# physiii/radio-mapper

Measured on AMD Instinct MI355X. Metric: IQ samples cross-correlated per second, higher is better.
Workload: dtype f32; 1 GPU; cfg3: 8 buoys (28 pairs), 10 MS/s complex64, N=4096-sample windows (L=8192), 4096 windows per GPU resident in HBM; n_buoys=8, n_pairs=28, n_samples=4096, windows_per_gpu=4096, channels=1, windows_total=4096, parallelism=windows sharded x1, no collective

## Files before the change

### radio-mapper_amd/csrc/host_plan.hpp

```cpp
#pragma once
#include <climits>
#include <cmath>
#include <cstdint>
#include <cstdio>
#include <cstring>
#include <map>
#include <mutex>
#include <string>
#include <vector>

namespace rmx {

struct PairItem {
    int i, j, out, run;
};

namespace host {

struct OptionSpec {
    const char* key;
    long lo, hi;
    const char* what;
};
inline const std::vector<OptionSpec>& option_specs() {
    static const std::vector<OptionSpec> s = {
        {"stag", 0, 5, "N = 4096 fused kernel: which waves run the two halves between barriers in the opposite order (default 1)"},
        {"ncus", 1, 4096, "persistent workgroups of the fused N = 4096 kernel (default: one per CU)"},
        {"chunk_windows", 1, 1 << 20, "windows per chunk of the unfused N = 4096 path"},
        {"small4096", 0, 1, "0: N = 4096 through the fused kernel however few the windows (default 1: few windows through the per-transform kernels)"},
        {"generic4096", 0, 1, "1: N = 4096 through the generic whole-window kernels instead of k_win"},
        {"small_maxl", 256, 16384, "largest zero-padded length that runs as one LDS transform per workgroup (default 8192)"},
        {"logl1", 4, 10, "four-step: log2 of the column length"},
        {"wfused", 0, 1, "0: never g_win_fused (<= 4 buoys, N = 256 ... 2048)"},
        {"wscr", 0, 2, "g_win_scr: 0 never, 2 also for batches that do not fill the chip"},
        {"wscr14", 0, 1, "0: N = 8192 with 1024 threads x one butterfly instead of 512 x two"},
        {"wscr_per_cu", 1, 8, "persistent g_win_scr workgroups per CU"},
        {"rows_anchor", 0, 64, "four-step inverse rows: 0 never g_rows_anchor, n = from n buoys on (default 6)"},
        {"fused", 0, 2, "four-step, <= 4 buoys: 0 always the two-kernel row passes, 2 g_rows_fused for any batch size"},
        {"fused_def", 0, 1, "0: the run-time pair loop of g_rows_fused also for the default plan"},
        {"gen_chunk", 1, 4096, "generic path: at most n windows per chunk of kernel launches"},
        {"rows_tpr", 1, 1024, "four-step: threads per row (selects the run-time-length row kernels)"},
        {"cols_threads", 64, 1024, "four-step: threads per column tile"},
        {"col_logt", 3, 5, "four-step: log2 columns per tile"},
        {"kwin16k", 0, 2, "N = 16384: 1 (default) k16_fwd + k16_pairs (four quarter transforms on the fused N = 4096 network) unless wscr = 2, 2 always, 0 g_win_eo15 / the four-step kernels"},
        {"k16_min_windows", 1, 1 << 30, "kwin16k = 1: smallest batch that takes k16_fwd / k16_pairs (default: 100 / (buoys + pairs), rounded up)"},
        {"kwin8k", 0, 2, "N = 8192, batches that fill the chip: 1 (default) k_win8kl (the bin-parity halves on the fused N = 4096 network, one anchor half in LDS), 0 g_win_scr14, 2 k_win8k (-DRMX_EXPERIMENTS builds only)"},
#ifdef RMX_EXPERIMENTS
        {"pk", 0, 1, "1: k_winp (packed fp32 build of the fused kernel; -DRMX_EXPERIMENTS builds only)"},
        {"win8", 0, 1, "1: k_win8 (8 points x 1024 threads; -DRMX_EXPERIMENTS builds only)"},
#endif
    };
    return s;
}

struct Knobs {
    std::map<std::string, long> v;
    bool get(const char* key, long* out) const {
        auto it = v.find(key);
        if (it == v.end()) return false;
        *out = it->second;
        return true;
    }
    long get_or(const char* key, long dflt) const {
        long x;
        return get(key, &x) ? x : dflt;
    }
};
inline std::mutex& knob_mutex() { static std::mutex m; return m; }
inline Knobs& default_knobs() { static Knobs k; return k; }

inline int set_default_option(const char* key, long value, std::string* err) {
    if (!key) { if (err) *err = "NULL key"; return -1; }
    for (const OptionSpec& s : option_specs()) {
        if (std::strcmp(s.key, key) != 0) continue;
        std::lock_guard<std::mutex> g(knob_mutex());
        if (value == LONG_MIN) { default_knobs().v.erase(key); return 0; }
        if (value < s.lo || value > s.hi) {
            if (err) { char b[160]; std::snprintf(b, sizeof b, "option '%s': %ld not in %ld..%ld", key, value, s.lo, s.hi); *err = b; }
            return -1;
// ... 45 lines not shown
    return kBandOk;
}

struct PairPlan {
    std::vector<int32_t> pairs;
    std::vector<PairItem> items;
    std::vector<int> part_begin;
    int n_parts = 0;
    bool all_pairs = false;
};

inline bool is_default_list(int n_buoys, const int32_t* pairs, int n_pairs) {
    if (n_pairs != (long)n_buoys * (n_buoys - 1) / 2) return false;
    int q = 0;
    for (int i = 0; pairs && i < n_buoys; ++i)
        for (int j = i + 1; j < n_buoys; ++j, ++q)
            if (pairs[2 * q] != i || pairs[2 * q + 1] != j) return false;
    return true;
}

inline int make_pair_plan(int n_buoys, const int32_t* pairs, int n_pairs, int pairs_per_block, PairPlan* out, std::string* err) {
    char b[200];
    const long all = (long)n_buoys * (n_buoys - 1) / 2;
    if (n_pairs < 0) { std::snprintf(b, sizeof b, "n_pairs %d < 0", n_pairs); *err = b; return -1; }
    std::vector<int32_t> pl;
    if (pairs) {
        pl.assign(pairs, pairs + 2 * (size_t)n_pairs);
    } else {
        if (n_pairs != all) { std::snprintf(b, sizeof b, "pairs == NULL needs n_pairs == %ld, got %d", all, n_pairs); *err = b; return -1; }
        pl.reserve(2 * (size_t)all);
        for (int i = 0; i < n_buoys; ++i)
            for (int j = i + 1; j < n_buoys; ++j) { pl.push_back(i); pl.push_back(j); }
    }
    for (int q = 0; q < n_pairs; ++q) {
        const int i = pl[2 * q], j = pl[2 * q + 1];
        if (i < 0 || j < 0 || i >= n_buoys || j >= n_buoys) {
            std::snprintf(b, sizeof b, "pair %d = (%d,%d) out of range for %d buoys", q, i, j, n_buoys);
            *err = b;
            return -1;
        }
    }
    out->items.resize(n_pairs);
    for (int q = 0; q < n_pairs; ++q) out->items[q] = PairItem{pl[2 * q], pl[2 * q + 1], q, 1};
    for (int q = n_pairs - 2; q >= 0; --q)
        if (out->items[q].i == out->items[q + 1].i) out->items[q].run = out->items[q + 1].run + 1;
    const int ppb = pairs_per_block > 0 ? pairs_per_block : 7;
    const int n_parts = n_pairs > 0 ? (n_pairs + ppb - 1) / ppb : 0;
    out->part_begin.assign(n_parts + 1, 0);
    for (int k = 0; k <= n_parts && n_parts > 0; ++k) out->part_begin[k] = (int)((long)k * n_pairs / n_parts);
    out->n_parts = n_parts;
    out->all_pairs = is_default_list(n_buoys, pl.data(), n_pairs);
    out->pairs.swap(pl);
    return 0;
}

inline long generic_chunk_windows(int n_buoys, long L, int max_windows, long budget_bytes, long cap) {
    const long all_pairs = (long)n_buoys * (n_buoys - 1) / 2;
    const long per_win = (long)(n_buoys + all_pairs) * L * 8;
    long chunk = per_win > 0 ? budget_bytes / per_win : 1;
    if (chunk < 1) chunk = 1;
    if (chunk > max_windows) chunk = max_windows;
    if (chunk > 4096) chunk = 4096;
    if (cap >= 1 && cap < chunk) chunk = cap;
    return chunk;
}

constexpr long kGenericBudgetBytes = 32L << 30;
constexpr long kGenericMaxChunk = 4096;
constexpr long kMaxGridY = 65535;
struct BandsPlan {
    long chunk = 0;
    long vwindows = 0;
    long slots = 0;
    size_t prod_bytes = 0;
    size_t rec_bytes = 0;
    size_t halo_bytes = 0;
    size_t out_elems = 0;
};
inline BandsPlan plan_bands(long chunk, long n_windows, int n_bands, int n_buoys, int n_pairs, long L, bool four_step, long col_tiles,
                            int logL1, size_t rec_size, long budget_bytes = kGenericBudgetBytes, long max_vwindows = kGenericMaxChunk) {
    BandsPlan b;
    const long nb = n_bands > 0 ? n_bands : 1, np = n_pairs > 0 ? n_pairs : 0;
    if (chunk < 1) chunk = 1;
    if (nb > 1) {
        if (chunk * nb > max_vwindows) chunk = max_vwindows / nb;
        if (four_step) {
            const long per_win = ((long)n_buoys + nb * np) * L * 8;
            if (per_win > 0 && chunk > budget_bytes / per_win) chunk = budget_bytes / per_win;
            if (np > 0 && chunk * nb * np > kMaxGridY) chunk = kMaxGridY / (nb * np);
        }
        if (chunk < 1) chunk = 1;
    }
    b.chunk = chunk;
    b.vwindows = chunk * nb;
    b.slots = b.vwindows * np;
    if (four_step) {
        b.prod_bytes = (size_t)b.slots * (size_t)L * 8;
        b.rec_bytes = (size_t)b.slots * (size_t)col_tiles * rec_size;
        b.halo_bytes = ((size_t)b.slots * (size_t)col_tiles * 2 * sizeof(float)) << logL1;
    }
    b.out_elems = (size_t)(n_windows > 0 ? n_windows : 0) * (size_t)nb * (size_t)np;
    return b;
}

inline double fused_cost4096(int n_cus, int n_buoys, int n_pairs, long n_windows) {
    const long cus = n_cus > 0 ? n_cus : 1;
// ... 155 lines not shown
```

### radio-mapper_amd/csrc/kwin.hpp

```cpp
#pragma once
#include <hip/hip_runtime.h>

#include <cmath>
#include <type_traits>
#include <vector>

#include "fft_r16.hpp"
#include "lag_bounds.hpp"

namespace rmx {

using u32x4 = unsigned int __attribute__((ext_vector_type(4)));
using u32x2 = unsigned int __attribute__((ext_vector_type(2)));
using f32x4 = float __attribute__((ext_vector_type(4)));
using f32x2 = float __attribute__((ext_vector_type(2)));

constexpr int kLdsXchg = kXchgF2 * 8;
constexpr int kLdsTw2 = 16 * kTw2RowF2 * 8;
constexpr int kLdsRed = 64;
constexpr int kLdsBytes = kLdsXchg + kLdsTw2 + kLdsRed;

__device__ __forceinline__ void load_tw2_to_lds(float2* tw2_lds, const float2* __restrict__ tw2_g, int t) {
    if (t < 256) tw2_lds[(t >> 4) * kTw2RowF2 + (t & 15)] = tw2_g[t];
}
// ... 41 lines not shown
    const int g = lane >> 3, r = lane & 7;
    const bool act = g < cnt;
    const int slot = (first + g) & (kResSlots - 1);
    const float* rf = reinterpret_cast<const float*>(red) + 4 * (slot * 8 + r);
    const int* ri = reinterpret_cast<const int*>(rf);
    const float ex = act ? rf[0] : -3.0f;
    const int k = act ? ri[1] : 0x7fffffff;
    const float tm = rf[2], tp = rf[3];
    const int out = oidx[slot];
    float gmax = ex;
    gmax = fmaxf(gmax, __builtin_bit_cast(float, dpp_i<0xB1>(__builtin_bit_cast(int, gmax))));
    gmax = fmaxf(gmax, __builtin_bit_cast(float, dpp_i<0x4E>(__builtin_bit_cast(int, gmax))));
    gmax = fmaxf(gmax, __builtin_bit_cast(float, dpp_i<0x141>(__builtin_bit_cast(int, gmax))));
    int kstar = (ex == gmax) ? k : 0x7fffffff;
    kstar = min(kstar, dpp_i<0xB1>(kstar));
    kstar = min(kstar, dpp_i<0x4E>(kstar));
    kstar = min(kstar, dpp_i<0x141>(kstar));
    const bool win = act && ex == gmax && k == kstar;
    auto halo_tap = [&](int kk) -> float {
        kk = kk < 0 ? 0 : (kk > 2 * kM - 2 ? 2 * kM - 2 : kk);
        int tt, q;
        k_to_owner(kk, tt, q);
        const int ln = tt & 63;
        const int row = ln < 2 ? ln : (ln >= 62 ? ln - 60 : 0);
        return halo[(((slot * 8 + (tt >> 6)) * kHaloRows) + row) * 16 + q];
    };
    const int kc = win ? k : (kM - 1);
    const float hm = halo_tap(kc - 1), hp = halo_tap(kc + 1);
    const float b = sqrtf(fmaxf(ex, 0.0f)) * out_scale;
    const float a = sqrtf(tm >= 0.0f ? tm : hm) * out_scale;
    const float c = sqrtf(tp >= 0.0f ? tp : hp) * out_scale;
    const double den = (double)a - 2.0 * (double)b + (double)c;
    float frac = 0.0f;
    if constexpr (BOUNDED) {
        int klo = 0, khi = 0;
        if (act) lag_window(lb, w, out, kM - 1, klo, khi);
        if (kc > klo && kc < khi && den != 0.0) frac = (float)(0.5 * ((double)a - (double)c) / den);
    } else {
        if (kc > 0 && kc < 2 * kM - 2 && den != 0.0) frac = (float)(0.5 * ((double)a - (double)c) / den);
    }
    if (win) {
        lag_int[obase + out] = kc - (kM - 1);
        lag_frac[obase + out] = frac;
        peak[obase + out] = b;
    }
}

template <bool U8>
__global__ __launch_bounds__(kThreads, 2) void k_win(const void* __restrict__ iq_v, float4* __restrict__ spec,
                                                     const float4* __restrict__ tw1_g,
                                                     const float2* __restrict__ tw2_g, int n_buoys,
                                                     long first_window, float out_scale,
                                                     int* __restrict__ lag_int, float* __restrict__ lag_frac,
                                                     float* __restrict__ peak, int n_win, int , int stag) {
    constexpr bool BOUNDED = false;
    constexpr LagBounds lb{nullptr, 0, 0, 0};
#include "kwin_body.hpp"
}

template <bool U8>
__global__ __launch_bounds__(kThreads, 2) void k_win_lb(const void* __restrict__ iq_v, float4* __restrict__ spec,
                                                        const float4* __restrict__ tw1_g,
                                                        const float2* __restrict__ tw2_g, int n_buoys,
                                                        long first_window, float out_scale,
                                                        int* __restrict__ lag_int, float* __restrict__ lag_frac,
                                                        float* __restrict__ peak, int n_win, int , int stag, LagBounds lb) {
    constexpr bool BOUNDED = true;
#include "kwin_body.hpp"
}

constexpr int kTw1ScaleLog2 = 6;
constexpr double kTw1Scale = 1.0 / (1 << kTw1ScaleLog2);
inline void build_tables(std::vector<float4>& tw1, std::vector<float2>& tw2) {
    const double two_pi = 6.283185307179586476925286766559;
    tw1.resize(8 * kThreads);
    std::vector<float2> t1(16 * kThreads);
    for (int t = 0; t < kThreads; ++t) {
        const int p = t & 1, u = t >> 1;
        for (int k0 = 0; k0 < 16; ++k0) {
            double ang = -two_pi * (double)((u * k0) % kM) / (double)kM;
            if (p) ang += -two_pi * (double)u / (double)kL;
            t1[k0 * kThreads + t] = make_float2((float)(std::cos(ang) * kTw1Scale), (float)(std::sin(ang) * kTw1Scale));
        }
    }
    for (int j = 0; j < 8; ++j)
        for (int t = 0; t < kThreads; ++t) {
            const float2 a = t1[(2 * j) * kThreads + t], b = t1[(2 * j + 1) * kThreads + t];
            tw1[j * kThreads + t] = make_float4(a.x, a.y, b.x, b.y);
        }
    tw2.resize(256);
    for (int a = 0; a < 16; ++a)
        for (int b = 0; b < 16; ++b) {
            const double ang = -two_pi * (double)((a * b) % 256) / 256.0;
            tw2[a * 16 + b] = make_float2((float)std::cos(ang), (float)std::sin(ang));
        }
}

}
```

### radio-mapper_amd/csrc/kwin_body.hpp

```cpp
    extern __shared__ __attribute__((aligned(16))) char smem[];
    float2* img0 = reinterpret_cast<float2*>(smem);
    float2* img1 = reinterpret_cast<float2*>(smem + kLdsWinImg);
    float2* tw2_lds = reinterpret_cast<float2*>(smem + kLdsWinTw2);
    float* halo = reinterpret_cast<float*>(smem + kLdsWinHalo);
    float4* red = reinterpret_cast<float4*>(smem + kLdsWinRed);
    int* oidx = reinterpret_cast<int*>(smem + kLdsWinOidx);

    const int t = threadIdx.x;
    const int p = t & 1, u = t >> 1;
    const int lane = t & 63, wave = t >> 6;
    const int B = n_buoys;
    const int n_pairs = B * (B - 1) / 2;

    load_tw2_to_lds_grouped(tw2_lds, tw2_g, t);
    float2 tw1[16];
    load_tw1(tw1, tw1_g, t);
    const float4* tw2row = reinterpret_cast<const float4*>(tw2_lds + (t & 15) * kTw2RowF2);
    const int loc_m0[2] = {__builtin_amdgcn_readfirstlane(wave * kLocWave),
                           __builtin_amdgcn_readfirstlane(kLdsWinImg + wave * kLocWave)};
    const int loc_rd = wave * kLocWave + loc_read_off(lane);
    const float sgn = p ? -1.0f : 1.0f;
    const int kbase = p ? (u - 1) : (u + kM - 1);
    const int hl = lane < 2 ? lane : lane - 60;
    const bool is_halo = lane < 2 || lane >= 62;
// ... 233 lines not shown
        }
        const int qsel = min(min(qa, qb), min(qc, qd));
        const int kq = kbase + qsel * 256;
        const int wi = __builtin_bit_cast(int, wrow);
        const float wmax = fmaxf(fmaxf(__builtin_bit_cast(float, __builtin_amdgcn_readlane(wi, 0)),
                                       __builtin_bit_cast(float, __builtin_amdgcn_readlane(wi, 16))),
                                 fmaxf(__builtin_bit_cast(float, __builtin_amdgcn_readlane(wi, 32)),
                                       __builtin_bit_cast(float, __builtin_amdgcn_readlane(wi, 48))));
        const unsigned long long hit = __ballot(tmax == wmax);
        int kw, ls, qs;
        if (__popcll(hit) == 1) {
            ls = __ffsll((long long)hit) - 1;
            kw = __builtin_amdgcn_readlane(kq, ls);
            qs = __builtin_amdgcn_readlane(qsel, ls);
        } else {
            kw = wave_min_i32(tmax == wmax ? kq : 0x7fffffff);
            int ts;
            k_to_owner(kw, ts, qs);
            ls = ts & 63;
        }
        typedef float f16v __attribute__((ext_vector_type(16)));
        const f16v mv = {mag[0], mag[1], mag[2],  mag[3],  mag[4],  mag[5],  mag[6],  mag[7],
                         mag[8], mag[9], mag[10], mag[11], mag[12], mag[13], mag[14], mag[15]};
        const float sel = mv[__builtin_amdgcn_readfirstlane(qs)];
        const int seli = __builtin_bit_cast(int, sel);
        const float tapm = ls >= 2 ? __builtin_bit_cast(float, __builtin_amdgcn_readlane(seli, ls >= 2 ? ls - 2 : 0)) : -2.0f;
        const float tapp = ls <= 61 ? __builtin_bit_cast(float, __builtin_amdgcn_readlane(seli, ls <= 61 ? ls + 2 : 63)) : -2.0f;
        if (lane == 0) {
            const u32x4 rec = {__float_as_uint(wmax), (unsigned)kw, __float_as_uint(tapm), __float_as_uint(tapp)};
            *reinterpret_cast<u32x4*>(red + rb * 8 + wave) = rec;
            if (wave == 0) oidx[rb] = out_idx;
        }
        ++npend;
        ++npair;
    };
    auto pair = [&](const C16& a, const C16& s, int out_idx, auto prefetch) __attribute__((always_inline)) {
        pair_h1(a, s, seq, prefetch);
        barrier_hook(false);
        pair_h2(seq, out_idx);
        ++seq;
    };
    auto out_of = [&](int i, int j) -> int { return i * B - (i * (i + 1)) / 2 + (j - i - 1); };

    load_x(sa, 0);
    if (B > 1) load_x(sb, 1);
    cvt_x(sa);
    fwd(sa);
    for (int e = 1; e + 1 < B; ++e) {
        cvt_x(sb);
        fwd(sb);
        store_spec(sb, e);
        pair(sa, sb, out_of(0, e), [&](auto part) __attribute__((always_inline)) { load_x_part(sb, e + 1, part); });
    }
    if (B > 1) {
        cvt_x(sb);
        fwd(sb);
        store_spec(sb, B - 1);
        pair(sa, sb, out_of(0, B - 1), [&](auto part) __attribute__((always_inline)) {
            if (B > 2) {
                load_spec_part(sa, 1, part);
                load_spec_part(sb, B - 1, part);
            }
        });
    }
    {
        const int M2 = (B - 1) * (B - 2) / 2;
        const bool late_h2 = stag == 1 ? ((wave >> 1) & 1) : stag == 2 ? (wave & 1) : stag == 3 ? (wave >> 2) :
                             stag == 4 ? ((wave ^ (wave >> 2)) & 1) : (stag == 5);
        auto j_of = [&](int i, int s) -> int { return (i & 1) ? (B - 1 - s) : (i + 1 + s); };
        int ci = 1, cs = 0;
        int ni = 1, ns = 1;
        if (ns >= B - 1 - ni) { ++ni; ns = 0; }
        auto h1_of = [&](int hi, int hs, int tr) __attribute__((always_inline)) {
            int pi = hi, ps = hs + 1;
            if (ps >= B - 1 - pi) { ++pi; ps = 0; }
            const bool valid = pi + 1 < B;
            const bool new_anchor = valid && pi != hi;
            const int pj = valid ? j_of(pi, ps) : B - 1;
            pair_h1(sa, sb, tr, [&](auto part) __attribute__((always_inline)) {
                if constexpr (decltype(part)::value == 0) {
                    if (new_anchor) {
                        load_spec_part(sa, pi, std::integral_constant<int, 0>{});
                        load_spec_part(sa, pi, std::integral_constant<int, 1>{});
                        load_spec_part(sa, pi, std::integral_constant<int, 2>{});
                        load_spec_part(sa, pi, std::integral_constant<int, 3>{});
                        load_spec_part(sa, pi, std::integral_constant<int, 4>{});
                        load_spec_part(sa, pi, std::integral_constant<int, 5>{});
                        load_spec_part(sa, pi, std::integral_constant<int, 6>{});
                        load_spec_part(sa, pi, std::integral_constant<int, 7>{});
                    }
                }
                load_spec_part(sb, pj, part);
            });
        };
        if (M2 > 0) h1_of(ci, cs, seq);
        for (int m = 0; m < M2; ++m) {
            barrier_hook(false);
            const bool has_next = m + 1 < M2;
            const int out_idx = out_of(ci, j_of(ci, cs));
            if (wave >= 4) __builtin_amdgcn_s_setprio(1);
            if (late_h2) {
                if (has_next) h1_of(ni, ns, seq + 1);
                if (wave >= 4) __builtin_amdgcn_s_setprio(0);
                pair_h2(seq, out_idx);
            } else {
                pair_h2(seq, out_idx);
                if (wave >= 4) __builtin_amdgcn_s_setprio(0);
                if (has_next) h1_of(ni, ns, seq + 1);
            }
            ++seq;
            ci = ni; cs = ns;
            ++ns;
            if (ns >= B - 1 - ni) { ++ni; ns = 0; }
        }
    }
    seq = 0;
    barrier_hook(true);
    }
```

### radio-mapper_amd/csrc/rmx_hip.hip

```cpp
#include <hip/hip_runtime.h>

#include <cmath>
#include <cstdarg>
#include <cstdio>
#include <cstdlib>
#include <cstring>
#include <new>
#include <string>
#include <type_traits>
#include <utility>
#include <vector>

#include "../../include/rmx.h"
#include "host_plan.hpp"
#include "lag_bounds.hpp"
#include "xspec_weight.hpp"
#include "xspec_bands.hpp"
#include "integrate.hpp"
#include "refine.hpp"
#include "quality.hpp"
#include "fft_r16.hpp"
#include "kwin.hpp"
#include "fft_r8.hpp"
#ifdef RMX_EXPERIMENTS
// ... 3 lines not shown
#include "generic_path.hpp"
#include "win_eo.hpp"
#include "pair4096.hpp"
#include "kwin8k.hpp"
#include "kwin16k.hpp"
#ifdef RMX_EXPERIMENTS
#include "../../tools/experiments/kwin8k.hpp"
#endif
#include "caf_select.hpp"
#include "solve_path.hpp"
#include "detect_path.hpp"

struct rmx_ctx {
    struct DevStage {
        int32_t* h = nullptr;  size_t h_elems = 0;
        int* d = nullptr;      size_t d_elems = 0;
        hipEvent_t ev = nullptr;
    };
    struct GenericKernels {
        decltype(&rmx::gen::g_cols_inv<4>) cols_inv = nullptr;
        decltype(&rmx::gen::g_cols_inv<4, 0, rmx::LagBounds>) cols_inv_lb = nullptr;
        decltype(&rmx::gen::g_cols_inv<4, 0, rmx::LagBounds, rmx::Integrate>) cols_inv_int = nullptr;
        decltype(&rmx::gen::g_cols_fwd<false, 4>) cols_fwd[2] = {nullptr, nullptr};
        decltype(&rmx::gen::g_rows<true, false>) rows_fwd = nullptr;
        decltype(&rmx::gen::g_rows<true, false, false, 0, rmx::XWeight>) rows_fwd_wt = nullptr;
        decltype(&rmx::gen::g_rows<false, true, true>) rows_inv = nullptr;
        decltype(&rmx::gen::g_rows<false, true, true, 0, rmx::BandSet>) rows_inv_bs = nullptr;
        decltype(&rmx::gen::g_rows_anchor<9>) rows_anchor = nullptr;
        decltype(&rmx::gen::g_rows_fused<2, 9>) fused = nullptr;
        decltype(&rmx::gen::g_rows_fused<2, 9>) fused_def = nullptr;
        decltype(&rmx::gen::g_win_fused<2, 9, false, false>) wf[2][2] = {{nullptr, nullptr}, {nullptr, nullptr}};
        size_t wf_lds[2] = {0, 0};
        decltype(&rmx::gen::g_win_scr<9, false>) ws[2] = {nullptr, nullptr};
        decltype(&rmx::gen::g_win_eo15<false>) ws15[2] = {nullptr, nullptr};
        size_t ws_lds = 0;
        int ws_thr = 0, ws_upw = 0;
    };

    rmx::host::Knobs knobs;
    int device = 0;
    int n_cus = 256;
    int n_buoys = 0, n_samples = 0, max_windows = 0;
    hipStream_t stream = nullptr;
    bool own_stream = false;
    int chunk_windows = 0;
    int pairs_per_block = 7;
    bool ppb_user = false;
    bool small_batch = true;
    bool timing = false;
    bool resident = true;
    int pk = 0;
    int win8 = 0;
    int stag = 1;
    float4* d_tw1_8 = nullptr;
    float2* d_tb8 = nullptr;
    float2* d_tc8 = nullptr;
    bool fused = true;
    float4* d_spec = nullptr;
    float4* d_tw1 = nullptr;
    float2* d_tw2 = nullptr;
    rmx::PairItem* d_items = nullptr;
    int* d_part_begin = nullptr;
    void* d_in = nullptr;      size_t d_in_bytes = 0;
    int* d_lag = nullptr;      float* d_frac = nullptr;  float* d_peak = nullptr;  size_t d_out_elems = 0;
    int* d_dop = nullptr;
    float* d_quality = nullptr;  size_t d_quality_elems = 0;
    void* h_out = nullptr;     size_t h_out_bytes = 0;
    size_t spec_bytes = 0, scratch_bytes = 0;
    bool generic = false;
    int g_logL = 0, g_logL1 = 0, g_logL2 = 0, g_lo_bits = 0, g_chunk = 0;
    size_t g_dyn_bytes = 0, g_pair_bytes = 0;
    GenericKernels gk;
    bool g_fused = false;
    bool g_fused_always = false;
    bool g_wfused = false;
    bool g_wscr = false;
    bool g_wscr_always = false;
    int g_ws_grid = 0;
    float4* g_ws_scratch = nullptr;
    float2* g_tw_win = nullptr;
    float2* g_tw_l = nullptr;
    bool g_k8 = false;
    int g_k8_kind = 1;
    float4* g_k8_tw1 = nullptr;
    float2* g_k8_tw2 = nullptr;
    int g_k16 = 0;
    float4* g_k16_tw1 = nullptr;
    float2 *g_k16_gq = nullptr, *g_k16_tw2 = nullptr, *g_k16_tws = nullptr;
    int g_rows_anchor_min_b = 6;
    float2 *g_tw = nullptr, *g_tw1 = nullptr, *g_tw2 = nullptr, *g_thi = nullptr, *g_tlo = nullptr;
    float2 *g_spec = nullptr, *g_spec_r = nullptr, *g_prod = nullptr;
    rmx::gen::GTile* g_rec = nullptr;
    float* g_halo = nullptr;
    rmx::gen::GPair* g_pairs = nullptr;
    long g_slots_alloc = 0;
    int g_pairs_n = -1;
    std::vector<int32_t> g_pairs_plan;
    hipStream_t copy_stream = nullptr;
    hipEvent_t copy_ev[4] = {nullptr, nullptr, nullptr, nullptr};
    float2* dt_tw = nullptr;  int dt_logn = 0;  float* dt_pdb = nullptr;  size_t dt_pdb_bytes = 0;
    void* dt_in = nullptr;  size_t dt_in_bytes = 0;  void* dt_out = nullptr;  size_t dt_out_bytes = 0;
    double* sv_buoys = nullptr;  int* sv_pairs = nullptr;  size_t sv_pairs_cap = 0;
    void* sv_in = nullptr;  size_t sv_in_bytes = 0;  void* sv_out = nullptr;  size_t sv_out_bytes = 0;
    float4* d_spec_r = nullptr;  size_t spec_r_bytes = 0;
    float2* caf_rot = nullptr;  size_t caf_rot_elems = 0;
    int* caf_lag = nullptr;  float* caf_frac = nullptr;  float* caf_peak = nullptr;  int* caf_dop = nullptr;
    size_t caf_out_elems = 0;
    float* caf_nb = nullptr;  size_t caf_nb_elems = 0;
    std::vector<double> caf_grid;
    DevStage lb_stage, band_stage;
    rmx::RefPair* rf_pairs = nullptr;
    std::vector<int32_t> rf_pairs_plan;
    std::vector<int32_t> plan_pairs;
// ... 959 lines not shown
    {
        std::string why;
        if (host::check_create_args(n_buoys, n_samples, max_windows, &why) != 0) return fail(nullptr, RMX_E_INVAL, "%s", why.c_str());
    }
    int ndev = rmx_device_count();
    if (ndev <= 0) return fail(nullptr, RMX_E_NODEV, "no HIP device visible");
    if (device_id < 0 || device_id >= ndev) return fail(nullptr, RMX_E_INVAL, "device_id %d not in 0..%d", device_id, ndev - 1);
    rmx_ctx* c = new (std::nothrow) rmx_ctx();
    if (!c) return fail(nullptr, RMX_E_NOMEM, "host allocation failed");
    c->knobs = host::snapshot_default_options();
    c->device = device_id;
    c->n_buoys = n_buoys;
    c->n_samples = n_samples;
    c->max_windows = max_windows;
    int rc = RMX_OK;
    auto bail = [&](int code) {
        g_create_error = c->err;
        rmx_destroy(c);
        return code;
    };
    auto init = [&]() -> int {
        RMX_HIP(c, hipSetDevice(device_id));
        {
            int ncu = 0;
            if (hipDeviceGetAttribute(&ncu, hipDeviceAttributeMultiprocessorCount, device_id) == hipSuccess && ncu > 0)
                c->n_cus = ncu;
            { long v; if (c->knobs.get("ncus", &v) && v > 0 && v < c->n_cus) c->n_cus = (int)v; }
        }
        RMX_HIP(c, hipStreamCreateWithFlags(&c->stream, hipStreamNonBlocking));
        c->own_stream = true;
        if (n_samples != kM || c->knobs.get_or("generic4096", 0) != 0) return rmx::generic_init(c);
        int chunk = (int)c->knobs.get_or("chunk_windows", 4096);
        if (chunk < 8) chunk = 8;
        chunk = (chunk + 7) & ~7;
        if (chunk > max_windows) chunk = max_windows;
        {
            const long per_win = (long)n_buoys * (8 * kThreads) * (long)sizeof(float4);
            const long cap = (8L << 30) / per_win;
            if (chunk > cap) chunk = (int)(cap > 8 ? (cap & ~7L) : 8);
        }
        c->chunk_windows = chunk;
        {
            const int wg = chunk < c->n_cus ? chunk : c->n_cus;
            c->spec_bytes = (size_t)wg * n_buoys * (8 * kThreads) * sizeof(float4);
        }
        RMX_HIP(c, hipMalloc((void**)&c->d_spec, c->spec_bytes));
        std::vector<float4> tw1;
        std::vector<float2> tw2;
        build_tables(tw1, tw2);
        RMX_HIP(c, hipMalloc((void**)&c->d_tw1, tw1.size() * sizeof(float4)));
        RMX_HIP(c, hipMalloc((void**)&c->d_tw2, tw2.size() * sizeof(float2)));
        RMX_HIP(c, hipMemcpy(c->d_tw1, tw1.data(), tw1.size() * sizeof(float4), hipMemcpyHostToDevice));
        RMX_HIP(c, hipMemcpy(c->d_tw2, tw2.data(), tw2.size() * sizeof(float2), hipMemcpyHostToDevice));
        c->scratch_bytes = c->spec_bytes + tw1.size() * sizeof(float4) + tw2.size() * sizeof(float2);
        c->stag = (int)c->knobs.get_or("stag", 1);
        c->small_batch = c->knobs.get_or("small4096", 1) != 0;
#ifdef RMX_EXPERIMENTS
        {
            std::vector<float4> t1;
            std::vector<float2> tb, tc;
            build_tables8(t1, tb, tc);
            RMX_HIP(c, hipMalloc((void**)&c->d_tw1_8, t1.size() * sizeof(float4)));
            RMX_HIP(c, hipMalloc((void**)&c->d_tb8, tb.size() * sizeof(float2)));
            RMX_HIP(c, hipMalloc((void**)&c->d_tc8, tc.size() * sizeof(float2)));
            RMX_HIP(c, hipMemcpy(c->d_tw1_8, t1.data(), t1.size() * sizeof(float4), hipMemcpyHostToDevice));
            RMX_HIP(c, hipMemcpy(c->d_tb8, tb.data(), tb.size() * sizeof(float2), hipMemcpyHostToDevice));
            RMX_HIP(c, hipMemcpy(c->d_tc8, tc.data(), tc.size() * sizeof(float2), hipMemcpyHostToDevice));
            c->scratch_bytes += t1.size() * sizeof(float4) + (tb.size() + tc.size()) * sizeof(float2);
            int rc_x = allow_lds(c, w8::kLdsWin8Bytes, w8::k_win8<false>, w8::k_win8<true>);
            if (rc_x == RMX_OK) rc_x = allow_lds(c, pk::kLdsWinpBytes, k_winp<false>, k_winp<true>);
            if (rc_x != RMX_OK) return rc_x;
            c->pk = (int)c->knobs.get_or("pk", 0);
            c->win8 = (int)c->knobs.get_or("win8", 0);
        }
#endif
        int rc_l = allow_lds(c, kLdsBytes, k_fwd<false>, k_fwd<true>, k_fwd<false, XWeight>, k_fwd<true, XWeight>, k_pair_str<>,
                             k_pair_str<LagBounds>, k_pair_str<BandSet>, k_pair_str<LagBounds, BandSet>);
        if (rc_l == RMX_OK)
            rc_l = allow_lds(c, kLdsResBytes, k_pair_res<>, k_pair_res<LagBounds>, k_pair_res<BandSet>, k_pair_res<LagBounds, BandSet>);
        if (rc_l == RMX_OK) rc_l = allow_lds(c, kLdsWinBytes, k_win<false>, k_win<true>, k_win_lb<false>, k_win_lb<true>);
        return rc_l;
    };
    rc = init();
    if (rc != RMX_OK) return bail(rc);
    *out = c;
    return RMX_OK;
}

void rmx_destroy(rmx_ctx* c) {
    if (!c) return;
    (void)hipSetDevice(c->device);
    if (c->stream) (void)hipStreamSynchronize(c->stream);
    for (hipEvent_t e : c->ev) (void)hipEventDestroy(e);
    for (void* p : {(void*)c->g_tw, (void*)c->g_tw1, (void*)c->g_tw2, (void*)c->g_thi, (void*)c->g_tlo, (void*)c->g_spec,
                    (void*)c->g_spec_r, (void*)c->g_prod, (void*)c->g_rec, (void*)c->g_halo, (void*)c->g_pairs,
                    (void*)c->g_ws_scratch, (void*)c->g_tw_win, (void*)c->g_tw_l, (void*)c->g_k8_tw1, (void*)c->g_k8_tw2,
                    (void*)c->g_k16_tw1, (void*)c->g_k16_gq, (void*)c->g_k16_tw2, (void*)c->g_k16_tws})
        if (p) (void)hipFree(p);
    if (c->copy_stream) (void)hipStreamDestroy(c->copy_stream);
    for (hipEvent_t e : c->copy_ev)
        if (e) (void)hipEventDestroy(e);
    for (void* p : {(void*)c->dt_tw, (void*)c->dt_pdb, c->dt_in, c->dt_out})
        if (p) (void)hipFree(p);
    for (void* p : {(void*)c->sv_buoys, (void*)c->sv_pairs, c->sv_in, c->sv_out})
        if (p) (void)hipFree(p);
    for (void* p : {(void*)c->d_spec_r, (void*)c->caf_rot, (void*)c->caf_lag, (void*)c->caf_frac, (void*)c->caf_peak,
                    (void*)c->caf_dop, (void*)c->caf_nb})
        if (p) (void)hipFree(p);
    if (c->d_spec) (void)hipFree(c->d_spec);
    if (c->d_tw1) (void)hipFree(c->d_tw1);
    if (c->d_tw2) (void)hipFree(c->d_tw2);
    for (void* p : {(void*)c->d_tw1_8, (void*)c->d_tb8, (void*)c->d_tc8})
        if (p) (void)hipFree(p);
    if (c->d_items) (void)hipFree(c->d_items);
    if (c->d_part_begin) (void)hipFree(c->d_part_begin);
    if (c->d_in) (void)hipFree(c->d_in);
    if (c->d_lag) (void)hipFree(c->d_lag);
    if (c->h_out) (void)hipHostFree(c->h_out);
    if (c->rf_pairs) (void)hipFree(c->rf_pairs);
    if (c->d_quality) (void)hipFree(c->d_quality);
    for (DevStage* s : {&c->lb_stage, &c->band_stage}) {
        if (s->d) (void)hipFree(s->d);
        if (s->h) (void)hipHostFree(s->h);
        if (s->ev) (void)hipEventDestroy(s->ev);
    }
    if (c->own_stream && c->stream) (void)hipStreamDestroy(c->stream);
    delete c;
}

int rmx_set_stream(rmx_ctx* c, void* hip_stream) {
    if (!c) return RMX_E_INVAL;
    RMX_HIP(c, hipSetDevice(c->device));
    if (c->stream) RMX_HIP(c, hipStreamSynchronize(c->stream));
    if (c->own_stream && c->stream) (void)hipStreamDestroy(c->stream);
    c->stream = (hipStream_t)hip_stream;
    c->own_stream = false;
    return RMX_OK;
}

int rmx_set_default_option(const char* key, long value) {
    std::string why;
    if (host::set_default_option(key, value, &why) != 0) return fail(nullptr, RMX_E_INVAL, "%s", why.c_str());
    return RMX_OK;
}

void rmx_clear_default_options(void) { host::clear_default_options(); }

int rmx_set_option(rmx_ctx* c, const char* key, long value) {
    if (!c || !key) return RMX_E_INVAL;
    if (!strcmp(key, "chunk_windows")) {
        if (c->generic) return RMX_OK;
        long chunk = value < 8 ? 8 : value;
        chunk = (chunk + 7) & ~7L;
        if (chunk > c->max_windows) chunk = c->max_windows;
        {
            const long per_win = (long)c->n_buoys * (8 * kThreads) * (long)sizeof(float4);
            const long cap = (8L << 30) / per_win;
            if (chunk > cap) chunk = cap > 8 ? (cap & ~7L) : 8;
        }
        c->chunk_windows = (int)chunk;
        return RMX_OK;
    }
    if (!strcmp(key, "pairs_per_block")) {
        if (value < 1 || value > 1 << 20) return fail(c, RMX_E_INVAL, "pairs_per_block %ld out of range", value);
        c->pairs_per_block = (int)value;
        c->ppb_user = true;
        return RMX_OK;
    }
    if (!strcmp(key, "dbg")) {
        return fail(c, RMX_E_UNSUPPORTED, "option 'dbg': the timing-only ablation build was removed");
    }
    if (!strcmp(key, "pk") || !strcmp(key, "win8")) {
#ifdef RMX_EXPERIMENTS
        (key[0] == 'p' ? c->pk : c->win8) = value != 0;
        return RMX_OK;
#else
        return fail(c, RMX_E_UNSUPPORTED, "option '%s' exists only in the -DRMX_EXPERIMENTS build (k_win8 / k_winp)", key);
#endif
    }
    if (!strcmp(key, "stag")) {
        if (value < 0 || value > 5) return fail(c, RMX_E_INVAL, "stag %ld not in 0..5", value);
        c->stag = (int)value;
        return RMX_OK;
    }
    if (!strcmp(key, "small4096")) {
        c->small_batch = value != 0;
        return RMX_OK;
    }
    if (!strcmp(key, "fused")) {
        c->fused = value != 0;
        return RMX_OK;
    }
    if (!strcmp(key, "resident")) {
        c->resident = value != 0;
        return RMX_OK;
    }
    if (!strcmp(key, "timing")) {
        c->timing = value != 0;
        return RMX_OK;
    }
    return fail(c, RMX_E_INVAL, "unknown option '%s'", key);
}

static int ensure_spec(rmx_ctx* c, long windows) {
    const size_t nb = (size_t)windows * c->n_buoys * (8 * kThreads) * sizeof(float4);
    if (nb <= c->spec_bytes) return RMX_OK;
    RMX_HIP(c, hipStreamSynchronize(c->stream));
    float4* nspec = nullptr;
    RMX_HIP(c, hipMalloc((void**)&nspec, nb));
    (void)hipFree(c->d_spec);
    c->d_spec = nspec;
    c->scratch_bytes += nb - c->spec_bytes;
    c->spec_bytes = nb;
    return RMX_OK;
}

static constexpr size_t kPackedOutMax = 256 * 1024;
static int ensure_out(rmx_ctx* c, size_t out_elems) {
    if (c->d_out_elems >= out_elems) return RMX_OK;
    if (c->d_lag) (void)hipFree(c->d_lag);
    c->d_lag = nullptr; c->d_frac = nullptr; c->d_peak = nullptr; c->d_out_elems = 0;
    const size_t stride = (out_elems + 63) & ~(size_t)63;
    RMX_HIP(c, hipMalloc((void**)&c->d_lag, 4 * stride * sizeof(float)));
    c->d_frac = reinterpret_cast<float*>(c->d_lag) + stride;
    c->d_peak = c->d_frac + stride;
    c->d_dop = reinterpret_cast<int*>(c->d_peak + stride);
    c->d_out_elems = out_elems;
    return RMX_OK;
}
static int fetch_out(rmx_ctx* c, size_t out_elems, int32_t* lag_int, float* lag_frac, float* peak, int32_t* dop = nullptr) {
    const size_t nb = out_elems * sizeof(float);
    const char* last = reinterpret_cast<char*>(dop ? (void*)c->d_dop : (void*)c->d_peak);
    const size_t span = (size_t)(last - reinterpret_cast<char*>(c->d_lag)) + nb;
    if (span <= kPackedOutMax) {
        if (c->h_out_bytes < span) {
// ... 139 lines not shown
            RMX_HIP(c, hipStreamWaitEvent(c->copy_stream, c->copy_ev[3], 0));
        } else {
            RMX_HIP(c, hipMemcpyAsync(c->d_in, iq, in_bytes, hipMemcpyHostToDevice, c->stream));
        }
        d_iq = c->d_in;
    }
    int* d_lag = lag_int;
    float *d_frac = lag_frac, *d_peak = peak;
    const size_t out_elems = (size_t)(n_windows / call.integ) * n_pairs * (size_t)rq.n_bands;
    if (!out_dev) {
        rc = ensure_out(c, out_elems);
        if (rc == RMX_OK && call.qualified()) rc = ensure_quality(c, 4 * out_elems);
        if (rc != RMX_OK) return rc;
        d_lag = c->d_lag; d_frac = c->d_frac; d_peak = c->d_peak;
        if (call.qualified()) call.quality = c->d_quality;
    }
    auto done = [&](int rc_k) -> int {
        if (rc_k != RMX_OK || out_dev) return rc_k;
        if (call.qualified())
            RMX_HIP(c, hipMemcpyAsync(req.quality, c->d_quality, 4 * out_elems * sizeof(float), hipMemcpyDeviceToHost, c->stream));
        return fetch_out(c, out_elems, lag_int, lag_frac, peak);
    };
    if (c->generic) return done(rmx::generic_batch(c, call, caps, rq, plan, d_iq, d_lag, d_frac, d_peak, u8));
    const bool k_win_route = plan.route == host::kRouteKWin;
    const long chunk_w = n_windows < c->chunk_windows ? n_windows : c->chunk_windows;
    rc = ensure_spec(c, k_win_route ? (chunk_w < c->n_cus ? chunk_w : c->n_cus) : chunk_w);
    if (rc != RMX_OK) return rc;
    if (!k_win_route) return done(run_chunks(c, call, caps, d_iq, 0, n_windows, plan.chunk, n_pairs, d_lag, d_frac, d_peak, u8));
    const float out_scale = out_scale4096();
    int n_sub = 0;
    for (int w0 = 0; w0 < n_windows; w0 += plan.chunk) {
        const int wc = (n_windows - w0 < plan.chunk) ? n_windows - w0 : plan.chunk;
        const int wtail = host::route_wtail4096(caps, plan, n_pairs, w0, wc);
        const int wf = wc - wtail;
        const int sub = plan.pipelined ? kHostSubChunk : (wf > 0 ? wf : 1);
        for (int s0 = 0; s0 < wf; s0 += sub) {
            const int sc = wf - s0 < sub ? wf - s0 : sub;
            const long wfirst = (long)w0 + s0;
            if (plan.pipelined) {
                const size_t off = (size_t)wfirst * c->n_buoys * c->n_samples * samp_bytes;
                const size_t nb = (size_t)sc * c->n_buoys * c->n_samples * samp_bytes;
                hipEvent_t ev = c->copy_ev[n_sub % 3];
                ++n_sub;
                RMX_HIP(c, hipMemcpyAsync((char*)c->d_in + off, (const char*)iq + off, nb, hipMemcpyHostToDevice,
                                          c->copy_stream));
                RMX_HIP(c, hipEventRecord(ev, c->copy_stream));
                RMX_HIP(c, hipStreamWaitEvent(c->stream, ev, 0));
            }
            const int wgrid = sc < c->n_cus ? sc : c->n_cus;
            rc = with_u8(u8, [&](auto U) {
                constexpr bool U8 = decltype(U)::value;
                auto go = [&](auto kern, auto... lb) {
                    return launch(c, kTkPair4096, kern, dim3(wgrid), dim3(kThreads), kLdsWinBytes, d_iq, c->d_spec, c->d_tw1, c->d_tw2,
                                  c->n_buoys, wfirst, out_scale, d_lag, d_frac, d_peak, sc, 0, c->stag, lb...);
                };
#ifdef RMX_EXPERIMENTS
                if (c->win8)
                    return launch(c, kTkPair4096, w8::k_win8<U8>, dim3(wgrid), dim3(w8::kT8), w8::kLdsWin8Bytes, d_iq, c->d_spec, c->d_tw1_8,
                                  c->d_tb8, c->d_tc8, c->n_buoys, wfirst, out_scale, d_lag, d_frac, d_peak, sc, c->stag);
                if (c->pk)
                    return launch(c, kTkPair4096, k_winp<U8>, dim3(wgrid), dim3(kThreads), pk::kLdsWinpBytes, d_iq, c->d_spec, c->d_tw1,
                                  c->d_tw2, c->n_buoys, wfirst, out_scale, d_lag, d_frac, d_peak, sc);
#endif
                return call.bounded() ? go(k_win_lb<U8>, call.lb) : go(k_win<U8>);
            });
            if (rc != RMX_OK) return rc;
        }
        if (wtail) {
            rc = run_chunks(c, call, caps, d_iq, w0 + wf, wtail, wtail, n_pairs, d_lag, d_frac, d_peak, u8);
            if (rc != RMX_OK) return rc;
        }
    }
    return done(RMX_OK);
}

static int check_weighted(rmx_ctx* c, int n_windows, const double* band_cps, int band_per_window, unsigned weighting,
                          std::vector<int32_t>* bins, bool* weighted) {
    if (weighting != RMX_WEIGHT_NONE && weighting != RMX_WEIGHT_PHAT)
        return fail(c, RMX_E_INVAL, "unknown weighting %u (RMX_WEIGHT_NONE = 0, RMX_WEIGHT_PHAT = 1)", weighting);
    const int rc = check_n_windows(c, n_windows);
    if (rc != RMX_OK) return rc;
    const int N = c->n_samples;
    const long rows = band_cps ? (band_per_window ? (long)n_windows : 1L) : 1L;
    bins->resize((size_t)(2 * rows));
    bool all_full = true;
    for (long r = 0; r < rows; ++r) {
        const double lo = band_cps ? band_cps[2 * r] : -0.5, hi = band_cps ? band_cps[2 * r + 1] : 0.5;
        const char* shared = band_per_window ? "" : " (one band shared by every window)";
        int32_t* s = bins->data() + 2 * r;
        const host::BandCheck bc = host::band_to_bins(lo, hi, N, &s[0], &s[1]);
        if (bc == host::kBandNoInterval)
            return fail(c, RMX_E_INVAL, "band of window %ld%s: [%g, %g] is not an interval inside [-0.5, 0.5] cycles per sample",
                        r, shared, lo, hi);
        if (bc == host::kBandNoBin)
            return fail(c, RMX_E_INVAL, "band of window %ld%s: [%g, %g] keeps no bin of the %ld-point transform", r, shared, lo,
                        hi, 2L * N);
        all_full = all_full && s[0] == -N && s[1] == N - 1;
    }
    *weighted = !(all_full && weighting == RMX_WEIGHT_NONE);
    return RMX_OK;
}

static int check_bounded(rmx_ctx* c, int n_windows, int n_pairs, int integrate, const int32_t* lag_bounds,
                         int bounds_per_window, long* rows, bool* bounded) {
    const int nm1 = c->n_samples - 1;
    *rows = bounds_per_window ? (long)(n_windows / integrate) * n_pairs : (long)n_pairs;
    bool all_full = true;
// ... 649 lines not shown
```

Before: 282.9 billion samples/s.

## Drive k_win pair loop from host-planned trail table reusing one resident spectrum

Replaces the in-kernel anchor/row pair enumeration with a host-planned pair order, a snake-like trail where each next pair shares one buoy with the current one. The order is encoded as an int4 table in device memory and read with lookahead. Each step then loads only one new spectrum into either register array, instead of reloading all eight parts of a new anchor when the row changes, which cuts redundant spectrum loads. It also changes the k_win default staggering to 0, and adds a small table read plus a branch on a uniform selector per step.

```diff
diff --git a/radio-mapper_amd/csrc/host_plan.hpp b/radio-mapper_amd/csrc/host_plan.hpp
--- a/radio-mapper_amd/csrc/host_plan.hpp
+++ b/radio-mapper_amd/csrc/host_plan.hpp
@@ -7,6 +7,7 @@
 #include <map>
 #include <mutex>
 #include <string>
+#include <utility>
 #include <vector>
 
 namespace rmx {
@@ -24,7 +25,7 @@
 };
 inline const std::vector<OptionSpec>& option_specs() {
     static const std::vector<OptionSpec> s = {
-        {"stag", 0, 5, "N = 4096 fused kernel: which waves run the two halves between barriers in the opposite order (default 1)"},
+        {"stag", 0, 5, "N = 4096 fused kernel: which waves run the two halves between barriers in the opposite order (0 nobody: the default; 1 SIMDs 1 and 3, 2 odd waves, 3 the second wave of every SIMD, 4 one wave of every SIMD, 5 everybody); k_win8 of the experiments build: default 1"},
         {"ncus", 1, 4096, "persistent workgroups of the fused N = 4096 kernel (default: one per CU)"},
         {"chunk_windows", 1, 1 << 20, "windows per chunk of the unfused N = 4096 path"},
         {"small4096", 0, 1, "0: N = 4096 through the fused kernel however few the windows (default 1: few windows through the per-transform kernels)"},
@@ -176,6 +177,122 @@
     out->all_pairs = is_default_list(n_buoys, pl.data(), n_pairs);
     out->pairs.swap(pl);
     return 0;
+}
+
+struct TrailStep {
+    int i, j;
+    int out_idx;
+    int xi_arr;
+    int load_arr;
+    int load_idx;
+    int reload;
+    int load2;
+};
+struct PairTrail {
+    int n_buoys = 0;
+    int first_load = -1;
+    std::vector<TrailStep> steps;
+    int loads = 0;
+    int reloads = 0, min_reloads = 0;
+    int sim_hits2 = 0, sim_hits3 = 0;
+};
+
+inline int trail_out_idx(int B, int i, int j) { return i * B - (i * (i + 1)) / 2 + (j - i - 1); }
+
+inline int trail_sim_hits(const PairTrail& t, int cap) {
+    std::vector<int> lru;
+    auto touch = [&](int b) -> bool {
+        bool hit = false;
+        for (size_t k = 0; k < lru.size(); ++k)
+            if (lru[k] == b) { lru.erase(lru.begin() + (long)k); hit = true; break; }
+        lru.insert(lru.begin(), b);
+        if ((int)lru.size() > cap) lru.pop_back();
+        return hit;
+    };
+    int hits = 0;
+    for (int b = 1; b < t.n_buoys; ++b) touch(b);
+    if (t.first_load >= 0) hits += touch(t.first_load);
+    for (const TrailStep& s : t.steps) {
+        if (s.load_idx >= 0) hits += touch(s.load_idx);
+        if (s.reload) hits += touch(s.load2);
+    }
+    return hits;
+}
+
+inline void trail_from_pairs(int B, const std::vector<std::pair<int, int>>& pairs, PairTrail* t) {
+    t->n_buoys = B;
+    t->steps.clear();
+    t->loads = t->reloads = 0;
+    t->first_load = -1;
+    if (pairs.empty()) return;
+    t->first_load = pairs[0].first == B - 1 ? pairs[0].second : pairs[0].first;
+    int arr_of[2] = {t->first_load, B - 1};
+    for (size_t k = 0; k < pairs.size(); ++k) {
+        const int a = pairs[k].first, b = pairs[k].second;
+        TrailStep s{};
+        s.i = a < b ? a : b;
+        s.j = a < b ? b : a;
+        s.out_idx = trail_out_idx(B, s.i, s.j);
+        s.xi_arr = arr_of[0] == s.i ? 0 : 1;
+        s.load_arr = 0; s.load_idx = -1; s.reload = 0; s.load2 = -1;
+        if (k + 1 < pairs.size()) {
+            const int c = pairs[k + 1].first, d = pairs[k + 1].second;
+            const bool keep_c = c == a || c == b, keep_d = d == a || d == b;
+            if (keep_c == keep_d) {
+                s.reload = 1;
+                s.load_arr = 0; s.load_idx = c < d ? c : d; s.load2 = c < d ? d : c;
+                arr_of[0] = s.load_idx; arr_of[1] = s.load2;
+                t->loads += 2;
+                ++t->reloads;
+            } else {
+                const int keep = keep_c ? c : d;
+                s.load_arr = arr_of[0] == keep ? 1 : 0;
+                s.load_idx = keep_c ? d : c;
+                arr_of[s.load_arr] = s.load_idx;
+                ++t->loads;
+            }
+        }
+        t->steps.push_back(s);
+    }
+    t->sim_hits2 = trail_sim_hits(*t, 2);
+    t->sim_hits3 = trail_sim_hits(*t, 3);
+}
+
+inline PairTrail plan_pair_trail(int B) {
+    PairTrail t;
+    t.n_buoys = B;
+    const int n = B - 1;
+    std::vector<std::pair<int, int>> pairs;
+    std::vector<int> order;
+    for (int r = n - 1; r >= 1; --r) order.push_back(r);
+    int anchor = n;
+    while (!order.empty()) {
+        for (int r : order) pairs.push_back({anchor, r});
+        anchor = order.back();
+        order.pop_back();
+        for (size_t a = 0, b = order.size(); a + 1 < b; ++a, --b) { const int x = order[a]; order[a] = order[b - 1]; order[b - 1] = x; }
+    }
+    trail_from_pairs(B, pairs, &t);
+    t.min_reloads = 0;
+    return t;
+}
+
+inline bool trail_kernel_ok(const PairTrail& t) {
+    for (const TrailStep& s : t.steps)
+        if (s.xi_arr != 0 || s.reload != 0) return false;
+    return true;
+}
+
+inline std::vector<int32_t> encode_pair_trail(const PairTrail& t) {
+    std::vector<int32_t> e;
+    if (!trail_kernel_ok(t)) return e;
+    const int B = t.n_buoys;
+    e.reserve(4 * (t.steps.size() + 1));
+    const int some = B > 1 ? B - 1 : 0;
+    e.insert(e.end(), {trail_out_idx(B, 0, B - 1), 0, t.first_load >= 0 ? t.first_load : some, 0});
+    for (const TrailStep& s : t.steps)
+        e.insert(e.end(), {s.out_idx, s.load_arr, s.load_idx >= 0 ? s.load_idx : some, 0});
+    return e;
 }
 
 inline long generic_chunk_windows(int n_buoys, long L, int max_windows, long budget_bytes, long cap) {
diff --git a/radio-mapper_amd/csrc/kwin.hpp b/radio-mapper_amd/csrc/kwin.hpp
--- a/radio-mapper_amd/csrc/kwin.hpp
+++ b/radio-mapper_amd/csrc/kwin.hpp
@@ -117,7 +117,7 @@
                                                      const float2* __restrict__ tw2_g, int n_buoys,
                                                      long first_window, float out_scale,
                                                      int* __restrict__ lag_int, float* __restrict__ lag_frac,
-                                                     float* __restrict__ peak, int n_win, int , int stag) {
+                                                     float* __restrict__ peak, int n_win, const int4* __restrict__ trail, int stag) {
     constexpr bool BOUNDED = false;
     constexpr LagBounds lb{nullptr, 0, 0, 0};
 #include "kwin_body.hpp"
@@ -129,7 +129,7 @@
                                                         const float2* __restrict__ tw2_g, int n_buoys,
                                                         long first_window, float out_scale,
                                                         int* __restrict__ lag_int, float* __restrict__ lag_frac,
-                                                        float* __restrict__ peak, int n_win, int , int stag, LagBounds lb) {
+                                                        float* __restrict__ peak, int n_win, const int4* __restrict__ trail, int stag, LagBounds lb) {
     constexpr bool BOUNDED = true;
 #include "kwin_body.hpp"
 }
diff --git a/radio-mapper_amd/csrc/kwin_body.hpp b/radio-mapper_amd/csrc/kwin_body.hpp
--- a/radio-mapper_amd/csrc/kwin_body.hpp
+++ b/radio-mapper_amd/csrc/kwin_body.hpp
@@ -309,66 +309,52 @@
         store_spec(sb, e);
         pair(sa, sb, out_of(0, e), [&](auto part) __attribute__((always_inline)) { load_x_part(sb, e + 1, part); });
     }
-    if (B > 1) {
-        cvt_x(sb);
-        fwd(sb);
-        store_spec(sb, B - 1);
-        pair(sa, sb, out_of(0, B - 1), [&](auto part) __attribute__((always_inline)) {
-            if (B > 2) {
-                load_spec_part(sa, 1, part);
-                load_spec_part(sb, B - 1, part);
-            }
-        });
-    }
     {
         const int M2 = (B - 1) * (B - 2) / 2;
+        const int4* __restrict__ tab = trail;
+        int4 cur = tab[0];
+        int4 nxt = tab[M2 > 0 ? 1 : 0];
+        if (B > 1) {
+            cvt_x(sb);
+            fwd(sb);
+            store_spec(sb, B - 1);
+            const int fl = cur.z;
+            pair(sa, sb, cur.x, [&](auto part) __attribute__((always_inline)) {
+                if (M2 > 0) load_spec_part(sa, fl, part);
+            });
+        }
+        auto h1_step = [&](const int4& st, int tr) __attribute__((always_inline)) {
+            const int li = st.z;
+            const int var = __builtin_amdgcn_readfirstlane(st.y);
+            int v0 = var, v1 = var;
+            asm volatile("" : "+s"(v0));
+            if (v0 == 0) pair_h1(sa, sb, tr, [&](auto part) __attribute__((always_inline)) { load_spec_part(sa, li, part); });
+            asm volatile("" : "+s"(v1));
+            if (v1 != 0) pair_h1(sa, sb, tr, [&](auto part) __attribute__((always_inline)) { load_spec_part(sb, li, part); });
+        };
         const bool late_h2 = stag == 1 ? ((wave >> 1) & 1) : stag == 2 ? (wave & 1) : stag == 3 ? (wave >> 2) :
                              stag == 4 ? ((wave ^ (wave >> 2)) & 1) : (stag == 5);
-        auto j_of = [&](int i, int s) -> int { return (i & 1) ? (B - 1 - s) : (i + 1 + s); };
-        int ci = 1, cs = 0;
-        int ni = 1, ns = 1;
-        if (ns >= B - 1 - ni) { ++ni; ns = 0; }
-        auto h1_of = [&](int hi, int hs, int tr) __attribute__((always_inline)) {
-            int pi = hi, ps = hs + 1;
-            if (ps >= B - 1 - pi) { ++pi; ps = 0; }
-            const bool valid = pi + 1 < B;
-            const bool new_anchor = valid && pi != hi;
-            const int pj = valid ? j_of(pi, ps) : B - 1;
-            pair_h1(sa, sb, tr, [&](auto part) __attribute__((always_inline)) {
-                if constexpr (decltype(part)::value == 0) {
-                    if (new_anchor) {
-                        load_spec_part(sa, pi, std::integral_constant<int, 0>{});
-                        load_spec_part(sa, pi, std::integral_constant<int, 1>{});
-                        load_spec_part(sa, pi, std::integral_constant<int, 2>{});
-                        load_spec_part(sa, pi, std::integral_constant<int, 3>{});
-                        load_spec_part(sa, pi, std::integral_constant<int, 4>{});
-                        load_spec_part(sa, pi, std::integral_constant<int, 5>{});
-                        load_spec_part(sa, pi, std::integral_constant<int, 6>{});
-                        load_spec_part(sa, pi, std::integral_constant<int, 7>{});
-                    }
+#pragma clang loop unroll(disable)
+        for (int m = 0; m <= M2; ++m) {
+            const int4 ahead = tab[m + 2 <= M2 ? m + 2 : M2];
+            if (m > 0) {
+                barrier_hook(false);
+                if (wave >= 4) __builtin_amdgcn_s_setprio(1);
+                if (!late_h2) {
+                    pair_h2(seq, cur.x);
+                    if (wave >= 4) __builtin_amdgcn_s_setprio(0);
                 }
-                load_spec_part(sb, pj, part);
-            });
-        };
-        if (M2 > 0) h1_of(ci, cs, seq);
-        for (int m = 0; m < M2; ++m) {
-            barrier_hook(false);
-            const bool has_next = m + 1 < M2;
-            const int out_idx = out_of(ci, j_of(ci, cs));
-            if (wave >= 4) __builtin_amdgcn_s_setprio(1);
-            if (late_h2) {
-                if (has_next) h1_of(ni, ns, seq + 1);
-                if (wave >= 4) __builtin_amdgcn_s_setprio(0);
-                pair_h2(seq, out_idx);
-            } else {
-                pair_h2(seq, out_idx);
-                if (wave >= 4) __builtin_amdgcn_s_setprio(0);
-                if (has_next) h1_of(ni, ns, seq + 1);
-            }
-            ++seq;
-            ci = ni; cs = ns;
-            ++ns;
-            if (ns >= B - 1 - ni) { ++ni; ns = 0; }
+            }
+            if (m < M2) h1_step(nxt, m > 0 ? seq + 1 : seq);
+            if (m > 0) {
+                if (late_h2) {
+                    if (wave >= 4) __builtin_amdgcn_s_setprio(0);
+                    pair_h2(seq, cur.x);
+                }
+                ++seq;
+            }
+            cur = nxt;
+            nxt = ahead;
         }
     }
     seq = 0;
diff --git a/radio-mapper_amd/csrc/rmx_hip.hip b/radio-mapper_amd/csrc/rmx_hip.hip
--- a/radio-mapper_amd/csrc/rmx_hip.hip
+++ b/radio-mapper_amd/csrc/rmx_hip.hip
@@ -79,6 +79,7 @@
     int pk = 0;
     int win8 = 0;
     int stag = 1;
+    int stag_kwin = 0;
     float4* d_tw1_8 = nullptr;
     float2* d_tb8 = nullptr;
     float2* d_tc8 = nullptr;
@@ -86,6 +87,7 @@
     float4* d_spec = nullptr;
     float4* d_tw1 = nullptr;
     float2* d_tw2 = nullptr;
+    int4* d_trail = nullptr;
     rmx::PairItem* d_items = nullptr;
     int* d_part_begin = nullptr;
     void* d_in = nullptr;      size_t d_in_bytes = 0;
@@ -1151,8 +1153,13 @@
         RMX_HIP(c, hipMalloc((void**)&c->d_tw2, tw2.size() * sizeof(float2)));
         RMX_HIP(c, hipMemcpy(c->d_tw1, tw1.data(), tw1.size() * sizeof(float4), hipMemcpyHostToDevice));
         RMX_HIP(c, hipMemcpy(c->d_tw2, tw2.data(), tw2.size() * sizeof(float2), hipMemcpyHostToDevice));
-        c->scratch_bytes = c->spec_bytes + tw1.size() * sizeof(float4) + tw2.size() * sizeof(float2);
+        const std::vector<int32_t> trail = host::encode_pair_trail(host::plan_pair_trail(n_buoys));
+        if (trail.empty()) return fail(c, RMX_E_INVAL, "k_win cannot walk the pair order planned for %d buoys", n_buoys);
+        RMX_HIP(c, hipMalloc((void**)&c->d_trail, trail.size() * sizeof(int32_t)));
+        RMX_HIP(c, hipMemcpy(c->d_trail, trail.data(), trail.size() * sizeof(int32_t), hipMemcpyHostToDevice));
+        c->scratch_bytes = c->spec_bytes + tw1.size() * sizeof(float4) + tw2.size() * sizeof(float2) + trail.size() * sizeof(int32_t);
         c->stag = (int)c->knobs.get_or("stag", 1);
+        c->stag_kwin = (int)c->knobs.get_or("stag", 0);
         c->small_batch = c->knobs.get_or("small4096", 1) != 0;
 #ifdef RMX_EXPERIMENTS
         {
@@ -1209,6 +1216,7 @@
     if (c->d_spec) (void)hipFree(c->d_spec);
     if (c->d_tw1) (void)hipFree(c->d_tw1);
     if (c->d_tw2) (void)hipFree(c->d_tw2);
+    if (c->d_trail) (void)hipFree(c->d_trail);
     for (void* p : {(void*)c->d_tw1_8, (void*)c->d_tb8, (void*)c->d_tc8})
         if (p) (void)hipFree(p);
     if (c->d_items) (void)hipFree(c->d_items);
@@ -1279,7 +1287,7 @@
     }
     if (!strcmp(key, "stag")) {
         if (value < 0 || value > 5) return fail(c, RMX_E_INVAL, "stag %ld not in 0..5", value);
-        c->stag = (int)value;
+        c->stag = c->stag_kwin = (int)value;
         return RMX_OK;
     }
     if (!strcmp(key, "small4096")) {
@@ -1525,7 +1533,7 @@
                 constexpr bool U8 = decltype(U)::value;
                 auto go = [&](auto kern, auto... lb) {
                     return launch(c, kTkPair4096, kern, dim3(wgrid), dim3(kThreads), kLdsWinBytes, d_iq, c->d_spec, c->d_tw1, c->d_tw2,
-                                  c->n_buoys, wfirst, out_scale, d_lag, d_frac, d_peak, sc, 0, c->stag, lb...);
+                                  c->n_buoys, wfirst, out_scale, d_lag, d_frac, d_peak, sc, (const int4*)c->d_trail, c->stag_kwin, lb...);
                 };
 #ifdef RMX_EXPERIMENTS
                 if (c->win8)
```

After: 290.1 billion samples/s (median of 6 runs). 2.6% higher.
